# angela000/DQNFlappyBird

Hardware: AMD Instinct MI355X
Metric: env steps/sec (whole node) + DQN grad-steps/sec, 80x80x4 batch=32 (higher is better)
Workload: dtype f32

## Files before the change

### dqnflappybird_amd/csrc/fb_qnet.hip

```cpp
#include <math.h>
#include <stdlib.h>
#include "fb_common.h"

#ifndef FK_ABL
#define FK_ABL 0
#endif
#ifndef BW_ABL
#define BW_ABL 0
#endif

namespace {

typedef float f32x16 __attribute__((ext_vector_type(16)));

constexpr int OFF_W1 = 0, OFF_B1 = 8192, OFF_W2 = 8224, OFF_B2 = 40992, OFF_W3 = 41056, OFF_B3 = 77920,
              OFF_WF1 = 77984;
constexpr int CONV_PARAMS = OFF_WF1;
#include "fb_head.h"
#include "fb_sampler.h"
#include "fb_gather.h"
constexpr int MAXTB = 256;


struct Slice { const float *params; const uint8_t *states; int s_off, count; const uint16_t *w1s; int fshift; };
// ... 1729 lines not shown
        if (DUEL) {
#pragma unroll
            for (int r = 0; r < PERV; r++) { const int i = tid + r * 512; if (i < cv) lw[2 * WQ + i] = tv[r]; }
        }
        __syncthreads();
        const int kl = k0 % 64;
#pragma unroll 8
        for (int k = 0; k < KC; k++) {
            const float xs = rdlane(x, kl + k), xqs = rdlane(xq, kl + k);
#pragma unroll
            for (int a = 0; a < AT; a++) {
                const int o = k * AN + (a < A ? a : 0) * N + il;
                lg[a] = fmaf(xs, lw[o], lg[a]);
                ns[a] = fmaf(xqs, lw[WQ + o], ns[a]);
            }
            if (DUEL) nv = fmaf(rdlane(xv, kl + k), lw[2 * WQ + k * N + il], nv);
        }
    }
#pragma unroll
    for (int a = 0; a < AT; a++) lg[a] += H.P[H.hoff.bq + (a < A ? a : 0) * N + il];
    float nq[AT], mean = 0.f;
#pragma unroll
    for (int a = 0; a < AT; a++) {
        const int o = (a < A ? a : 0) * N + il;
        nq[a] = draw(LQ.eout + o) * (ns[a] + H.sig[H.off.bq + o]);
        if (a < A) mean += nq[a];
    }
    if (DUEL) {
        mean /= (float)A;
        const float vn = draw(LV.eout + il) * (nv + H.sig[H.off.bv + il]);
#pragma unroll
        for (int a = 0; a < AT; a++) lg[a] += (vn + nq[a]) - mean;
    } else {
#pragma unroll
        for (int a = 0; a < AT; a++) lg[a] += nq[a];
    }
    float qv[AT];
    const float z = H.sup.vmin + (float)(on ? lane : 0) * H.sup.dz;
    c51_q<AT>(lg, on, z, qv);
    if (lane == 0 && live) {
#pragma unroll
        for (int a = 0; a < AT; a++) if (a < A) H.q[(size_t)smp * A + a] = qv[a];
        int best = 0;
#pragma unroll
        for (int a = 1; a < AT; a++) if (a < A && qv[a] > qv[best]) best = a;
        const fb_u4 o = fb_philox(H.seed_lo, H.seed_hi, (uint32_t)key, H.step_lo, H.stream, H.step_hi);
        const float u = (float)(o.x >> 8) * (1.0f / 16777216.0f);
        if (u <= H.epsilon) best = (int)(((unsigned long long)o.y * (unsigned)A) >> 32);
        H.actions[smp] = (uint8_t)best;
    }
}

typedef float f32x4 __attribute__((ext_vector_type(4)));
struct FkArgs { Slices sl; const float *h3; float *hf; float *qpart; int FC, A, dueling, stot; NetOff off; };
constexpr int FK_ROW = 204;

__global__ __launch_bounds__(512) void fc1_fk_kernel(FkArgs a) {
    __shared__ float ast[8 * 16 * FK_ROW];
    __shared__ float red[8 * 4 * 64];
    const Slice s = a.sl.s[blockIdx.z];
    const int M = s.count, m0 = blockIdx.x * 16, n0 = blockIdx.y * 16;
    if (m0 >= M) return;
    const int lane = threadIdx.x & 63, wave = threadIdx.x >> 6, r = lane & 15, g = lane >> 4;
    const int kw = wave * 200;
    const float *bcol = s.params + OFF_WF1 + (size_t)(kw + 50 * g) * a.FC + n0 + r;
    float bv[50];
#pragma unroll
    for (int t = 0; t < 50; t++) bv[t] = bcol[(size_t)(FK_ABL == 2 ? 0 : t) * a.FC];
    float hb = s.params[a.off.bf1 + n0 + r], hw[MAXA + 1];
#pragma unroll
    for (int c = 0; c < MAXA; c++) hw[c] = s.params[a.off.wq + (n0 + r) * a.A + (c < a.A ? c : 0)];
    hw[MAXA] = s.params[(a.dueling ? a.off.wv : a.off.bf1) + n0 + r];
    float *mine = ast + wave * 16 * FK_ROW;
    float4 st[13];
#pragma unroll
    for (int i = 0; i < 13; i++) {
        const int idx = lane + 64 * i, row = idx < 800 ? idx / 50 : 0, c4 = idx < 800 ? idx - row * 50 : 0;
        const int mr = m0 + row < M ? m0 + row : M - 1;
        st[i] = *reinterpret_cast<const float4 *>(a.h3 + (size_t)(s.s_off + mr) * 1600 + kw + 4 * (FK_ABL == 3 ? 0 : c4));
    }
#pragma unroll
    for (int i = 0; i < 13; i++) {
        const int idx = lane + 64 * i, row = idx / 50, c4 = idx - row * 50;
        if (idx < 800) *reinterpret_cast<float4 *>(mine + row * FK_ROW + 4 * c4) = st[i];
    }
    __builtin_amdgcn_wave_barrier();
    asm volatile("s_waitcnt lgkmcnt(0)" ::: "memory");
    const float *arow = mine + r * FK_ROW + 50 * g;
    f32x4 acc0 = {0.f, 0.f, 0.f, 0.f}, acc1 = {0.f, 0.f, 0.f, 0.f};
    float2 av[25];
#pragma unroll
    for (int t = 0; t < 25; t++) av[t] = *reinterpret_cast<const float2 *>(arow + 2 * t);
#pragma unroll
    for (int t = 0; t < 25; t++) { keep(av[t].x); keep(av[t].y); }
#pragma unroll
    for (int t = 0; t < (FK_ABL == 1 ? 1 : 25); t++) {
        acc0 = __builtin_amdgcn_mfma_f32_16x16x4f32(rbf(av[t].x, a.sl.rb), rbf(bv[2 * t], a.sl.rb), acc0, 0, 0, 0);
        acc1 = __builtin_amdgcn_mfma_f32_16x16x4f32(rbf(av[t].y, a.sl.rb), rbf(bv[2 * t + 1], a.sl.rb), acc1, 0, 0, 0);
    }
#pragma unroll
    for (int q = 0; q < 4; q++) red[(wave * 4 + q) * 64 + lane] = acc0[q] + acc1[q];
    __syncthreads();
    if (threadIdx.x >= 256) return;
    const int reg = threadIdx.x >> 6, row = 4 * g + reg, col = r, mr = m0 + row, unit = n0 + col;
    float v = red[reg * 64 + lane];
#pragma unroll
    for (int w = 1; w < 8; w++) v += red[(w * 4 + reg) * 64 + lane];
    const bool live = mr < M;
    const size_t srow = (size_t)s.s_off + (live ? mr : M - 1);
    if (live) a.hf[srow * a.FC + unit] = v;
    if (!a.qpart || FK_ABL == 4) return;
    const float h = fmaxf(v + hb, 0.f);
    const int qs = a.A + 1;
    float *qo = a.qpart + (srow * (size_t)gridDim.y + blockIdx.y) * qs;
#pragma unroll
    for (int c = 0; c <= MAXA; c++) {
        if (c < a.A || (c == a.A && a.dueling)) {
            float x = h * (c == a.A ? hw[MAXA] : hw[c]);
#pragma unroll
            for (int o = 8; o > 0; o >>= 1) x += __shfl_xor(x, o, 16);
            if (col == 0 && live) qo[c] = x;
        }
    }
}

struct Bw1Args {
    int algo, B, FC, A, dueling, stot, n_dx, rb;
    NetOff off;
    const float *params, *pnext, *ptarget;
    const float *hf, *qpart, *h3;
    const uint8_t *act; const float *rew; const uint8_t *term; const float *isw;
    double gamma;
    float *grad, *dh3, *loss, *abs_err, *y_out;
    AdamDev *adam; int tick;
    FbGate gate;
};
constexpr int BW_DX_ROW = 4;
constexpr int BW_DW_ROW = 36;

template <int AT, bool DX, bool MD = false, bool DP = false, bool HU = false>
__device__ __forceinline__ void fc1_bwd2_body(const Bw1Args &L, float *smem, const MdPar M = MdPar{}, const float delta = 0.f) {
    const int tid = threadIdx.x, lane = tid & 63, wave = tid >> 6, B = L.B, FC = L.FC, A = AT == MAXA ? L.A : AT;
    const float *P = L.params;
    float (*dadv)[MAXA] = reinterpret_cast<float (*)[MAXA]>(smem);
    float *dv = smem + MAXTB * MAXA, *lterm = dv + MAXTB, *dadv2 = lterm + MAXTB, *big = dadv2 + 2 * MAXTB;
    const bool lead = blockIdx.x == 0;
    const bool dbl = DP || L.algo == FB_ALGO_DOUBLE;
    const bool row3 = MD || dbl;
    const int qs = A + 1, ntile = FC >> 4;
    constexpr bool dx_role = DX;
    const int mt = dx_role ? blockIdx.x / 50 : 0, t2 = dx_role ? 0 : blockIdx.x - L.n_dx, nt = t2 / 7, kg = t2 - nt * 7;
    const int kt = dx_role ? blockIdx.x - mt * 50 : kg * 8 + wave;
    auto unit_params = [&](int n, float &bias, float (&wq)[AT], float &wv) {
        bias = P[L.off.bf1 + n];
        wv = P[(L.dueling ? L.off.wv : L.off.bf1) + n];
#pragma unroll
        for (int c = 0; c < AT; c++) wq[c] = P[L.off.wq + n * A + (c < A ? c : 0)];
    };
    float pre_hf[32], pre_bias, pre_wq[AT], pre_wv, pre_a[16];
    float4 pre_w[8];
    if constexpr (DX) {
        const int ch = FC < 512 ? FC : 512, n = tid < ch ? tid : 0;
#pragma unroll
        for (int q = 0; q < 32; q++) { const int bq_ = mt * 32 + q; pre_hf[q] = L.hf[(size_t)(bq_ < B ? bq_ : 0) * FC + n]; }
        unit_params(n, pre_bias, pre_wq, pre_wv);
        const int kh = ch / 16, nbeg = wave * (ch / 8) + (lane >> 5) * kh;
        const float *brun = P + OFF_WF1 + (size_t)(kt * 32 + (lane & 31)) * FC + nbeg;
#pragma unroll
        for (int q = 0; q < 8; q++) pre_w[q] = *reinterpret_cast<const float4 *>(brun + (4 * q < kh ? 4 * q : 0));
#pragma unroll
        for (int q = 0; q < 16; q++) pre_a[q] = 0.f;
#pragma unroll
        for (int q = 0; q < 2; q++) { const int mr = mt * 32 + drow(2 * (wave & 7) + q, lane); pre_a[q] = L.h3[(size_t)(mr < B ? mr : 0) * 1600 + kt * 32 + (lane & 31)]; }
    } else {
        const int c = tid & 31;
#pragma unroll
        for (int q = 0; q < 2; q++) { const int b = (tid >> 5) + 16 * q; pre_hf[q] = L.hf[(size_t)(b < B ? b : 0) * FC + nt * 32 + c]; }
#pragma unroll
        for (int q = 2; q < 32; q++) pre_hf[q] = 0.f;
        unit_params(nt * 32 + c, pre_bias, pre_wq, pre_wv);
        const int ktc = kt < 50 ? kt : 0;
#pragma unroll
        for (int t = 0; t < 16; t++) { const int b = 2 * t + (lane >> 5); pre_a[t] = L.h3[(size_t)(b < B ? b : 0) * 1600 + ktc * 32 + (lane & 31)]; }
#pragma unroll
        for (int q = 0; q < 8; q++) pre_w[q] = make_float4(0.f, 0.f, 0.f, 0.f);
    }
    float bqs[AT], bqn[AT], bq3[AT];
#pragma unroll
    for (int c = 0; c < AT; c++) { const int cc = c < A ? c : 0; bqs[c] = L.params[L.off.bq + cc]; bqn[c] = L.pnext[L.off.bq + cc]; bq3[c] = L.ptarget[L.off.bq + cc]; }
    const int bvo = L.dueling ? L.off.bv : L.off.bq;
    float bvs = L.params[bvo], bvn = L.pnext[bvo], bv3 = L.ptarget[bvo];
    for (int b0 = 0; b0 < (BW_ABL == 1 ? 0 : B); b0 += 32) {
        const int b = b0 + (tid >> 4), j = tid & 15, bc = b < B ? b : 0;
        float rf = L.rew[bc], isw = L.isw ? L.isw[bc] : 1.f;
        int termb = L.term[bc], a_b = L.act[bc];
        float x0[2][AT + 1], x1[2][AT + 1], x2[2][AT + 1];
#pragma unroll
        for (int u = 0; u < 2; u++) {
            const int tile = j + 16 * u, tc = tile < ntile ? tile : 0;
            const float *q0 = L.qpart + ((size_t)bc * ntile + tc) * qs;
            const size_t rs = (size_t)ntile * qs;
#pragma unroll
            for (int c = 0; c <= AT; c++) {
                const int cc = c < qs ? c : 0;
                x0[u][c] = q0[cc]; x1[u][c] = q0[(size_t)B * rs + cc]; x2[u][c] = q0[(size_t)(row3 ? 2 * B : 0) * rs + cc];
            }
        }
        keep(rf); keep(isw); keep(termb); keep(a_b);
        float qsv[AT + 1], qnv[AT + 1], q3v[AT + 1];
#pragma unroll
        for (int c = 0; c <= AT; c++) {
            keep(x0[0][c]); keep(x1[0][c]); keep(x2[0][c]); keep(x0[1][c]); keep(x1[1][c]); keep(x2[1][c]);
            const bool on = c < A || (c == A && L.dueling), on0 = on && j < ntile, on1 = on && j + 16 < ntile;
            qsv[c] = (on0 ? x0[0][c] : 0.f) + (on1 ? x0[1][c] : 0.f);
            qnv[c] = (on0 ? x1[0][c] : 0.f) + (on1 ? x1[1][c] : 0.f);
            q3v[c] = (on0 ? x2[0][c] : 0.f) + (on1 ? x2[1][c] : 0.f);
        }
        for (int tile = j + 32; tile < ntile; tile += 16) {
            const float *q0 = L.qpart + ((size_t)bc * ntile + tile) * qs;
            const size_t rs = (size_t)ntile * qs;
#pragma unroll
            for (int c = 0; c <= AT; c++) {
                const int cc = c < qs ? c : 0;
                const bool on = c < A || (c == A && L.dueling);
                const float y0 = q0[cc], y1 = q0[(size_t)B * rs + cc], y2 = q0[(size_t)(row3 ? 2 * B : 0) * rs + cc];
                qsv[c] += on ? y0 : 0.f; qnv[c] += on ? y1 : 0.f; q3v[c] += on ? y2 : 0.f;
            }
        }
#pragma unroll
        for (int c = 0; c <= AT; c++)
#pragma unroll
            for (int o = 8; o > 0; o >>= 1) { qsv[c] += __shfl_xor(qsv[c], o, 16); qnv[c] += __shfl_xor(qnv[c], o, 16); q3v[c] += __shfl_xor(q3v[c], o, 16); }
// ... 11 lines not shown
        };
        fin(qsv, vs, bqs, bvs);
        fin(qnv, vn, bqn, bvn);
        fin(q3v, v3, bq3, bv3);
        float sel;
        {
            int am = 0;
#pragma unroll
            for (int c = 1; c < AT; c++) if (c < A && qnv[c] > qnv[am]) am = c;
            float seld = q3v[0], selm = qnv[0];
#pragma unroll
            for (int c = 1; c < AT; c++) { seld = c == am ? q3v[c] : seld; selm = c < A ? fmaxf(selm, qnv[c]) : selm; }
            sel = dbl ? seld : selm;
        }
        if (L.algo != FB_ALGO_PER) isw = 1.f;
        double rr = rf == 0.1f ? 0.1 : (double)rf;
        if constexpr (MD) {
            float bonus;
            mdqn_target<AT>(qnv, q3v, A, a_b, M, sel, bonus);
            rr += (double)bonus;
        }
        const double yd = termb ? rr : rr + L.gamma * (double)sel;
        const float y = (float)yd;
        float qe = qsv[0];
#pragma unroll
        for (int c = 1; c < AT; c++) qe = c == a_b ? qsv[c] : qe;
        const float d = y - qe;
        const float scale = L.algo == FB_ALGO_DQN ? 2.f : 2.f / (float)B;
        const float gq = -scale * isw * td_clamp<HU>(d, delta);
        const bool pg = L.algo == FB_ALGO_PG;
        float pgp[AT], pgl;
        {
            float mx = qsv[0], se = 0.f;
#pragma unroll
            for (int c = 1; c < AT; c++) mx = c < A ? fmaxf(mx, qsv[c]) : mx;
#pragma unroll
            for (int c = 0; c < AT; c++) { pgp[c] = c < A ? expf(qsv[c] - mx) : 0.f; se += pgp[c]; }
#pragma unroll
            for (int c = 0; c < AT; c++) pgp[c] /= se;
            pgl = logf(se) - (qe - mx);
        }
        const float pgw = rf / (float)L.gamma;
        if (j == 0 && b < B) {
            lterm[b] = pg ? pgl * pgw : td_term<HU>(isw, d, delta);
            if (lead && L.abs_err) L.abs_err[b] = fabsf(d);
            if (lead && L.y_out) L.y_out[b] = y;
            dv[b] = L.dueling && !pg ? gq : 0.f;
#pragma unroll
            for (int c = 0; c < AT; c++) dadv[b][c] = pg ? (pgp[c] - (c == a_b ? 1.f : 0.f)) * pgw : (c == a_b ? gq : 0.f) - (L.dueling ? gq / (float)A : 0.f);
            if (AT == 2) { dadv2[2 * b] = dadv[b][0]; dadv2[2 * b + 1] = dadv[b][1]; }
        }
    }
#pragma unroll
    for (int q = 0; q < 32; q++) keep(pre_hf[q]);
#pragma unroll
    for (int q = 0; q < 16; q++) keep(pre_a[q]);
#pragma unroll
    for (int q = 0; q < 8; q++) { keep(pre_w[q].x); keep(pre_w[q].y); keep(pre_w[q].z); keep(pre_w[q].w); }
    __syncthreads();
    if (lead && tid == 0) {
        float sum = 0.f;
        for (int b = 0; b < B; b++) sum += lterm[b];
        *L.loss = L.algo == FB_ALGO_DQN || L.algo == FB_ALGO_PG ? sum : sum / (float)B;
        adam_tick(L.adam, L.tick);
    }
    if (lead && tid >= 64 && tid < 64 + A) { const int c = tid - 64; float sum = 0.f; for (int b = 0; b < B; b++) sum += dadv[b][c]; L.grad[L.off.bq + c] = sum; }
    if (lead && tid == 128 && L.dueling) { float sum = 0.f; for (int b = 0; b < B; b++) sum += dv[b]; L.grad[L.off.bv] = sum; }
    auto dhf_of = [&](int b, float hfv, float bias, const float (&wq)[AT], float wv, float &hout) {
        const float v = hfv + bias;
        float d = L.dueling ? dv[b] * wv : 0.f;
#pragma unroll
        for (int c = 0; c < AT; c++) if (c < A) d = fmaf(dadv[b][c], wq[c], d);
        hout = fmaxf(v, 0.f);
        return v > 0.f ? d : 0.f;
    };
    const int hl = lane >> 5, i = lane & 31, jj = lane & 31;
    if constexpr (DX) {
        const int RS = 512 + BW_DX_ROW;
        float *dh = big, *red = big + 32 * RS;
        f32x16 acc = {0};
        for (int nc = 0; nc < FC; nc += 512) {
            const int ch = FC - nc < 512 ? FC - nc : 512;
            if (nc) {
                __syncthreads();
                const int n = nc + (tid < ch ? tid : 0);
#pragma unroll
                for (int q = 0; q < 32; q++) { const int bq_ = mt * 32 + q; pre_hf[q] = L.hf[(size_t)(bq_ < B ? bq_ : 0) * FC + n]; }
                unit_params(n, pre_bias, pre_wq, pre_wv);
                const int kh = ch / 16, nbeg = wave * (ch / 8) + hl * kh;
                const float *brun = P + OFF_WF1 + (size_t)(kt * 32 + jj) * FC + nc + nbeg;
#pragma unroll
                for (int q = 0; q < 8; q++) pre_w[q] = *reinterpret_cast<const float4 *>(brun + (4 * q < kh ? 4 * q : 0));
            }
            if (tid < ch && BW_ABL != 2) {
                if (AT == 2 && !L.dueling) {
                    float4 da[16];
#pragma unroll
                    for (int q = 0; q < 16; q++) da[q] = *reinterpret_cast<const float4 *>(dadv2 + 2 * (mt * 32 + 2 * q < MAXTB - 1 ? mt * 32 + 2 * q : 0));
                    float o[32];
#pragma unroll
                    for (int q = 0; q < 16; q++) {
                        const float v0 = pre_hf[2 * q] + pre_bias, v1 = pre_hf[2 * q + 1] + pre_bias;
                        const float d0 = fmaf(da[q].y, pre_wq[1], fmaf(da[q].x, pre_wq[0], 0.f)), d1 = fmaf(da[q].w, pre_wq[1], fmaf(da[q].z, pre_wq[0], 0.f));
                        o[2 * q] = (v0 > 0.f && mt * 32 + 2 * q < B) ? d0 : 0.f;
                        o[2 * q + 1] = (v1 > 0.f && mt * 32 + 2 * q + 1 < B) ? d1 : 0.f;
                    }
#pragma unroll
                    for (int q = 0; q < 32; q++) dh[q * RS + tid] = o[q];
                } else {
#pragma unroll
                    for (int q = 0; q < 32; q++) {
                        float hv;
                        dh[q * RS + tid] = mt * 32 + q < B ? dhf_of(mt * 32 + q, pre_hf[q], pre_bias, pre_wq, pre_wv, hv) : 0.f;
                    }
                }
            }
            __syncthreads();
            const int kh = ch / 16, nbeg = wave * (ch / 8) + hl * kh;
            const float *arun = dh + i * RS + nbeg;
            float4 xa[8];
#pragma unroll
            for (int q = 0; q < 8; q++) xa[q] = *reinterpret_cast<const float4 *>(arun + (4 * q < kh ? 4 * q : 0));
#pragma unroll
            for (int q = 0; q < 8; q++) { keep(xa[q].x); keep(xa[q].y); keep(xa[q].z); keep(xa[q].w); }
#pragma unroll
            for (int q = 0; q < 8; q++) {
                if (4 * q < kh && BW_ABL != 3) {
                    const float4 x = xa[q], w = pre_w[q];
                    const bool rb = L.rb;
                    acc = mfma(rbf(x.x, rb), rbf(w.x, rb), acc); acc = mfma(rbf(x.y, rb), rbf(w.y, rb), acc);
                    acc = mfma(rbf(x.z, rb), rbf(w.z, rb), acc); acc = mfma(rbf(x.w, rb), rbf(w.w, rb), acc);
                }
            }
        }
        reduce_rows<8>(acc, red, wave, lane, mt * 32, B, [&](float v, int r, int mr) {
            const size_t o = (size_t)mr * 1600 + kt * 32 + jj;
            L.dh3[o] = BW_ABL == 4 ? v : (((r & 1) ? pre_a[1] : pre_a[0]) > 0.f ? v : 0.f);
        });
        return;
    }
    if (BW_ABL == 5) return;
    float *dh = big, *hh = big + MAXTB * BW_DW_ROW;
    {
        const int c = tid & 31;
#pragma unroll
        for (int q = 0; q < 2; q++) {
            const int b = (tid >> 5) + 16 * q;
            if (b < B) { float hv; dh[b * BW_DW_ROW + c] = dhf_of(b, pre_hf[q], pre_bias, pre_wq, pre_wv, hv); hh[b * BW_DW_ROW + c] = hv; }
        }
        for (int b = (tid >> 5) + 32; b < B; b += 16) {
            float hv;
            dh[b * BW_DW_ROW + c] = dhf_of(b, L.hf[(size_t)b * FC + nt * 32 + c], pre_bias, pre_wq, pre_wv, hv);
            hh[b * BW_DW_ROW + c] = hv;
        }
    }
    __syncthreads();
    if (kt < 50) {
        f32x16 acc = {0};
#pragma unroll
        for (int t = 0; t < 16; t++) {
            const int b = 2 * t + hl;
            const float w = dh[(b < B ? b : 0) * BW_DW_ROW + jj];
            acc = mfma(b < B ? rbf(pre_a[t], L.rb) : 0.f, b < B ? rbf(w, L.rb) : 0.f, acc);
        }
#pragma unroll 4
        for (int t = 16; t < (B + 1) / 2; t++) {
            const int b = 2 * t + hl, bc = b < B ? b : 0;
// ... 1135 lines not shown
        }
    }
    if (bid == ADAMF_T2 + ADAMF_T3 && tid == 0) { a.ad->applies = a.ad->ticks; a.ad->pver[0] += 1; a.ad->wverc[0] = a.ad->pver[0]; }
    if (bid == ADAMF_T2 + ADAMF_T3 && tid < (int)(a.n & 3)) {
        const long long q = (n4 << 2) + tid;
        float mm = a.m[q], vv = a.v[q];
        mm += (a.g[q] - mm) * omb1; vv += (a.g[q] * a.g[q] - vv) * omb2;
        a.p[q] -= (mm * alpha) / (sqrtf(vv) + eps);
        a.m[q] = mm; a.v[q] = vv;
    }
    if (a.split && bid == ADAMF_T2 + ADAMF_T3 && tid == 0) fb_flag_wait(&a.split->env_done, a.split_val, &a.split->timeouts[4]);
}

__global__ void init_params_kernel(float *__restrict__ p, long long n, NetOff off, int FC, int A, int dueling,
                                   uint32_t seed_lo, uint32_t seed_hi) {
    const long long i = (long long)blockIdx.x * blockDim.x + threadIdx.x;
    if (i >= n) return;
    bool bias = (i >= OFF_B1 && i < OFF_W2) || (i >= OFF_B2 && i < OFF_W3) || (i >= OFF_B3 && i < OFF_WF1) ||
                (i >= off.bf1 && i < off.bf1 + FC) || (i >= off.bq && i < off.bq + A) || (dueling && i == off.bv);
    if (bias) { p[i] = 0.01f; return; }
    for (uint32_t ctr = 0;; ctr++) {
        const fb_u4 r = fb_philox(seed_lo, seed_hi, (uint32_t)i, ctr, FB_STREAM_INIT, 0u);
        const float u1 = ((r.x >> 8) + 1) * (1.0f / 16777216.0f), u2 = (r.y >> 8) * (1.0f / 16777216.0f);
        const float z = sqrtf(-2.f * logf(u1)) * cosf(6.28318530717958647692f * u2);
        if (fabsf(z) <= 2.f) { p[i] = 0.01f * z; return; }
    }
}

}

#ifndef FB_ADAM_GRID
#define FB_ADAM_GRID 1024
#endif
constexpr int ADAM_GRID = FB_ADAM_GRID;

#include <vector>
struct fb_qnet {
    std::vector<void *> allocs;
    int arch, FC, A, max_batch;
    long long n;
    NetOff off;
    float *params[2], *adam_m, *adam_v, *grad, *slabs;
    float *slabs1;
    uint16_t *w1s[2];
    uint4 *wsp[2];
    uint16_t *zeros;
    uint16_t *a1s, *a3s;
    int nsplit;
    int nsplit_train;
    bool adam_ticked;
    AdamDev *adam;
    float *p1, *h2, *h3, *hf, *q;
    float *qpart;
    unsigned long long *ring_fo;
    hipEvent_t grad_ev;
    hipEvent_t grad_ev_recorded;
    uint8_t *amax;
    float *dhf, *dh3, *dh2, *dp1;
    float *gmax;
    int zmax;
    float *hf_act, *hp_act;
    FbSplitCtx *split;
    C51Sup sup;
    float kappa;
    MdPar md;
    float huber;
    float *c51_dl, *c51_xs, *c51_lt;
    NetOff hoff;
    float *heff[2];
    bool noisy;
    long long ntot;
    NoisyNet nnet;
    float *mst[2], *nz[2];
    int act_noise;
    float *nz_zero, *ht;
    uint4 *wsig;
    uint16_t *a3n;
    int *sig_seen;
    bool split_adam_pending;
    float max_grad_norm;
    double *clip_part;
    float *clip_out;
    float ac_cv, ac_ce;
    float ppo_eps, ppo_vclip;
    float *ac_dl, *ac_xs, *ac_r;
    uint8_t *ac_t;
    SacOff sac_off;
    float sac_hbar, sac_alr;
    float *sac_w;
    IqnOff iqn_off;
    int iqn_n, iqn_np, iqn_k;
    float iqn_eta;
    float *iqn_dpre, *iqn_ctab;
    int iqn_mu;
    MdPar iqn_md;
    float *ppo_sum;
};

static NetOff make_off(int FC, int A, int dueling) {
    NetOff o;
    o.bf1 = OFF_WF1 + 1600 * FC;
    int p = o.bf1 + FC;
    if (dueling) { o.wv = p; o.bv = p + FC; p = o.bv + 1; } else { o.wv = 0; o.bv = 0; }
    o.wq = p; o.bq = p + FC * A; o.n = o.bq + A;
    return o;
}
// ... 190 lines not shown
                        : make_off(fc_width, sup.N ? n_actions * sup.N : n_actions, arch == FB_ARCH_DUELING || arch == FB_ARCH_AC || arch == FB_ARCH_IQN_DUELING);
    if (is_sac(h)) {
        h->sac_off.wq1 = h->off.n; h->sac_off.bq1 = h->sac_off.wq1 + fc_width * n_actions;
        h->sac_off.wq2 = h->sac_off.bq1 + n_actions; h->sac_off.bq2 = h->sac_off.wq2 + fc_width * n_actions;
        h->off.n = h->sac_off.bq2 + n_actions;
        h->sac_hbar = 0.98f * logf((float)n_actions); h->sac_alr = 0.f;
    }
    if (is_iqn(h)) {
        h->iqn_off.we = h->off.n; h->iqn_off.be = h->iqn_off.we + FB_IQN_COS * fc_width;
        h->off.n = h->iqn_off.be + fc_width;
        h->iqn_n = s.n_tau; h->iqn_np = s.n_tau_next; h->iqn_k = s.n_tau_act; h->iqn_eta = 1.f;
        h->iqn_mu = 0; h->iqn_md = MdPar{0.03f, 0.9f, -1.f};
    }
    h->hoff = is_c51d(h) ? make_off(fc_width, n_actions * sup.N, 0) : is_iqnd(h) ? make_off(fc_width, n_actions, 0) : h->off;
    h->n = h->off.n;
    h->noisy = s.noisy;
    h->ntot = h->noisy ? 2 * h->n - OFF_WF1 : h->n;
    if (h->noisy) h->nnet = make_noisy(h->off, arch, fc_width, n_actions, sup.N, s.sigma0);
    h->zmax = 64;
    const size_t S = (size_t)3 * max_batch, nb = sizeof(float) * (size_t)h->n, nbt = sizeof(float) * (size_t)h->ntot;
    hipError_t e = hipSuccess;
    auto alloc = [&](auto **p, size_t bytes) {
        void *q = nullptr;
        if (e == hipSuccess) e = hipMalloc(&q, bytes);
        if (e != hipSuccess) return;
        h->allocs.push_back(q);
        *p = static_cast<std::remove_reference_t<decltype(**p)> *>(q);
        e = hipMemset(q, 0, bytes);
    };
    alloc(&h->params[0], nb); alloc(&h->params[1], nb);
    alloc(&h->adam_m, nbt); alloc(&h->adam_v, nbt); alloc(&h->grad, nbt);
    if (h->noisy) for (int w = 0; w < 2; w++) { alloc(&h->mst[w], nbt); alloc(&h->nz[w], sizeof(float) * (size_t)h->nnet.nz); }
    if (h->noisy) {
        alloc(&h->nz_zero, sizeof(float) * (size_t)h->nnet.nz);
        alloc(&h->wsig, sizeof(uint4) * (size_t)wsp_w3t(fc_width));
        alloc(&h->a3n, S * 1600 * 6 + 256);
        alloc(&h->ht, S * fc_width * 4 * FC1_SP_KS);
        alloc(&h->sig_seen, sizeof(int));
        if (e == hipSuccess) e = hipMemset(h->sig_seen, 0xff, sizeof(int));
    }
    alloc(&h->slabs, sizeof(float) * (size_t)h->zmax * CONV_PARAMS);
    if (2 * max_batch > h->zmax) alloc(&h->slabs1, sizeof(float) * (size_t)2 * (max_batch < MAXTB ? max_batch : MAXTB) * CONV1_PARAMS);
    alloc(&h->adam, sizeof(AdamDev));
    alloc(&h->w1s[0], 3 * 8192 * 2); alloc(&h->w1s[1], 3 * 8192 * 2);
    const size_t wsp_bytes = (size_t)wsp_total(fc_width) * sizeof(uint4);
    alloc(&h->wsp[0], wsp_bytes); alloc(&h->wsp[1], wsp_bytes);
    h->nsplit = 3; h->nsplit_train = 3;
    alloc(&h->zeros, 256);
    alloc(&h->a1s, S * 3200 * 6); alloc(&h->a3s, S * 1600 * 6 + 256);
    alloc(&h->p1, S * 3200 * 4); alloc(&h->amax, S * 3200);
    alloc(&h->h2, S * 1600 * 4); alloc(&h->h3, S * 1600 * 4);
    alloc(&h->hf, S * fc_width * 4 * FC1_KS); alloc(&h->q, S * MAXA * 4);
    alloc(&h->qpart, (size_t)(fc_width / 16) * S * (MAXA + 1) * 4);
    alloc(&h->ring_fo, (size_t)max_batch * 4 * sizeof(unsigned long long));
    const size_t Bm = max_batch;
    alloc(&h->dhf, Bm * fc_width * 4); alloc(&h->dh3, Bm * 1600 * 4);
    alloc(&h->dh2, Bm * 1600 * 4); alloc(&h->dp1, Bm * 3200 * 4);
    alloc(&h->gmax, (size_t)(fc_width / 16) * 4);
    alloc(&h->hf_act, S * fc_width * 4 * FC1_SP_KS); alloc(&h->hp_act, sizeof(float) * (size_t)(h->n - h->off.bf1));
    if (sup.N) { alloc(&h->c51_dl, Bm * 64 * 4); alloc(&h->c51_xs, Bm * fc_width * 4); alloc(&h->c51_lt, Bm * 4); }
    if (is_c51d(h) || is_iqn(h)) for (int w = 0; w < 2; w++) alloc(&h->heff[w], sizeof(float) * (size_t)(h->hoff.n - h->off.bf1));
    if (is_ac(h)) {
        const size_t Bt = Bm < MAXTB ? Bm : MAXTB;
        alloc(&h->ac_dl, Bt * 16 * 4); alloc(&h->ac_xs, Bt * fc_width * 4); alloc(&h->ac_r, Bt * 4); alloc(&h->ac_t, Bt);
        alloc(&h->ppo_sum, 6 * 4);
    }
    if (is_sac(h)) {
        const size_t Bt = Bm < MAXTB ? Bm : MAXTB;
        alloc(&h->ac_dl, Bt * 16 * 4); alloc(&h->ac_xs, Bt * fc_width * 4); alloc(&h->sac_w, 8 * 4);
    }
    if (is_iqn(h)) {
        const size_t Bt = Bm < MAXTB ? Bm : MAXTB;
        alloc(&h->ac_dl, Bt * 4 * 4); alloc(&h->ac_xs, Bt * fc_width * 4);
        alloc(&h->iqn_dpre, Bt * h->iqn_n * fc_width * 4); alloc(&h->iqn_ctab, Bt * h->iqn_n * FB_IQN_COS * 4);
    }
    alloc(&h->clip_part, sizeof(double) * 256); alloc(&h->clip_out, sizeof(float) * 2);
    if (e == hipSuccess) { const float one = 1.f; e = hipMemcpy(h->clip_out + 1, &one, sizeof(one), hipMemcpyHostToDevice); }
    int rc = e == hipSuccess ? FB_OK : fb_set_error(e == hipErrorOutOfMemory ? FB_ERR_NOMEM : FB_ERR_HIP, "fb_qnet_create: %s", hipGetErrorString(e));
    if (rc == FB_OK) {
        AdamDev a; memset(&a, 0, sizeof(a));
        a.pver[0] = a.pver[1] = 1;
        if (hipMemcpy(h->adam, &a, sizeof(a), hipMemcpyHostToDevice) != hipSuccess) rc = fb_set_error(FB_ERR_HIP, "fb_qnet_create: hipMemcpy failed");
    }
    if (rc == FB_OK) rc = fb_qnet_set_hparams(h, 1e-6f, 0.9f, 0.999f, 1e-8f);
    if (rc == FB_OK && is_sac(h)) rc = sac_write_words(h, 0.2f);
    if (rc != FB_OK) { fb_qnet_destroy(h); return rc; }
    *out = h;
    return FB_OK;
}

extern "C" int fb_qnet_destroy(fb_qnet_t h) {
    if (!h) return FB_OK;
    if (h->split) {
        FbSplitCtx *c = h->split;
        if (c->tstream) { (void)hipStreamSynchronize(c->tstream); (void)hipStreamDestroy(c->tstream); }
        if (c->f) (void)hipFree(c->f);
        delete c;
    }
    for (void *p : h->allocs) (void)hipFree(p);
    delete h;
    return FB_OK;
}

__global__ void flag_wait_kernel(const unsigned long long *flag, unsigned long long v, unsigned *timeouts) { if (threadIdx.x == 0) fb_flag_wait(flag, v, timeouts); }
__global__ void flag_set_kernel(unsigned long long *flag, unsigned long long v) { fb_flag_store(flag, v); }

// ... 286 lines not shown
    if (p.train) { side.p1 = h->p1; side.amax = h->amax; }
    const int t1p = (rows * 100 + 7) / 8, gsp = min(256, (t1p + C1_WAVES - 1) / C1_WAVES);
    if (!c.trunk && !c.state_trunk && !c.fused && runs(c, K_CONV1))
        hipLaunchKernelGGL(conv1_sp_kernel, dim3(gsp), dim3(64 * C1_WAVES), 0, c.st, sl, (const uint8_t *)h->zeros, h->a1s, c.pl1, c.nsp, h->wsp[which], h->FC, pver, (const unsigned *)wver, side, &h->adam->ovf);
    C23Args c23{h->a1s + (size_t)row0 * 3200, c.pl1, h->wsp[which] + WSP_W2, s0.params + OFF_B2, s0.params + OFF_B3, h->a3s + (size_t)row0 * 1600, c.pl2, rows, pver, wver, c.only < 0 ? &h->adam->wverc[which] : nullptr,
                p.train ? h->h2 + (size_t)row0 * 1600 : nullptr, p.train ? h->h3 + (size_t)row0 * 1600 : nullptr,
                s0.states, s0.w1s, s0.params + OFF_B1, s0.params, h->wsp[which], h->FC, &h->adam->ovf};
    Fc1Args af{h->a3s + (size_t)row0 * 1600, c.pl2, h->zeros, h->wsp[which] + WSP_WF1, (c.fused ? h->hf_act : h->hf) + (size_t)row0 * h->FC, c.stot, rows, h->FC,
               c.fused ? pver : nullptr, c.fused ? wver : nullptr, nullptr, 0,
               c.fused ? head_base(h, s0.params) + h->off.bf1 : nullptr, c.fused ? h->hp_act : nullptr, c.fused ? (int)(h->hoff.n - h->off.bf1) : 0,
               c.fused && p.split && c.only < 0 ? &p.split->f->trunk_done : nullptr, p.split ? p.split->seq : 0};
    if (c.trunk && z1 < p.ns && rows % 128 == 0) {
        int z2 = z1 + 1;
        while (z2 < p.ns && p.sl.s[z2].params == p.sl.s[z1].params && p.sl.s[z2].s_off == p.sl.s[z2 - 1].s_off + p.sl.s[z2 - 1].count) z2++;
        const Slice sn = p.sl.s[z1];
        if (z2 == p.ns && sn.s_off == row0 + rows && sn.params != s0.params) {
            int rows2 = 0;
            for (int z = z1; z < z2; z++) rows2 += p.sl.s[z].count;
            af.w2 = h->wsp[sn.params == h->params[1] ? 1 : 0] + WSP_WF1; af.m_split = rows; af.M = rows + rows2;
            z1 = z2;
        }
    }
    *z = z1;
    const dim3 gc((rows + 4) / 5), gf(((af.M + 127) / 128) * (h->FC / 64) * FC1_SP_KS);
    if (c.fused && p.split && c.only < 0 && gc.x > 256 && gc.x % 256 != 0) { c23.round_flag = &p.split->f->last_round; c23.round_val = p.split->seq; c23.round_blk = (int)(gc.x / 256) * 256; }
    with_nsp(c.nsp, [&](auto ns) {
        if (!c.trunk && !c.state_trunk && runs(c, K_CONV2))
            with_bool(c.fused, [&](auto fu) { hipLaunchKernelGGL((conv23_sp_kernel<decltype(ns)::value, 5, decltype(fu)::value>), gc, dim3(512), 0, c.st, c23); });
        if (runs(c, K_FC1)) hipLaunchKernelGGL(fc1_sp_kernel<decltype(ns)::value>, gf, dim3(256), 0, c.st, af);
    });
    if (c.fused && (c.only < 0 || c.only == K_FC1) && (long long)af.hp_n > (long long)gf.x * 256) {
        const size_t done = (size_t)gf.x * 256;
        FB_CHECK_HIP(hipMemcpyAsync(h->hp_act + done, af.hp_src + done, sizeof(float) * ((size_t)af.hp_n - done), hipMemcpyDeviceToDevice, c.st));
    }
    return FB_OK;
}

static void small_trunk(fb_qnet *h, const Plan &p, const PlanCtx &c, bool planes) {
    SplitJob job;
    C23T c23t = trunk_args(h, p, c, &job);
    if (planes) { c23t.a3s = h->a3s; c23t.pl3 = c.pl2; }
    const int t1 = (c.maxc * 100 + 7) / 8;
    if (runs(c, K_CONV1))
        with_bool(p.nib, [&](auto nib) { hipLaunchKernelGGL(conv1_pool_kernel<decltype(nib)::value>, dim3((t1 + 3) / 4, 1, p.ns), dim3(256), 0, c.st, p.sl, h->p1, h->amax, job); });
    if (runs(c, K_CONV2))
        with_nsp(c.nsp, [&](auto ns) { hipLaunchKernelGGL((conv23_t_kernel<decltype(ns)::value, false>), dim3(c.maxc, p.ns), dim3(512), 0, c.st, c23t); });
}

static void small_forward(fb_qnet *h, const Plan &p, const PlanCtx &c) {
    if (!c.trunk) small_trunk(h, p, c, false);
    if (runs(c, K_FC1)) {
        FkArgs fa;
        fa.sl = p.sl; fa.h3 = h->h3; fa.hf = h->hf; fa.qpart = p.train && !c.c51 && !c.ac ? h->qpart : nullptr; fa.FC = h->FC; fa.A = h->A;
        fa.dueling = h->arch == FB_ARCH_DUELING; fa.stot = c.stot; fa.off = h->off;
        hipLaunchKernelGGL(fc1_fk_kernel, dim3((c.maxc + 15) / 16, h->FC / 16, p.ns), dim3(512), 0, c.st, fa);
    }
}

static void launch_dist_head(const fb_qnet *h, const C51HeadArgs &H, int rows, hipStream_t st) {
    with_actions(h->A, [&](auto a) {
        if (is_qr(h)) hipLaunchKernelGGL(qr_head_kernel<decltype(a)::value>, dim3((rows + 3) / 4), dim3(256), 0, st, H);
        else hipLaunchKernelGGL(c51_head_kernel<decltype(a)::value>, dim3((rows + 3) / 4), dim3(256), 0, st, H);
    });
}

static void head_stage(fb_qnet *h, const Plan &p, const PlanCtx &c) {
    auto shared = [&](auto &H) {
        H.hf = c.fused ? h->hf_act : h->hf; H.stot = c.stot; H.nks = c.big ? FC1_SP_KS : 1; H.FC = h->FC; H.A = h->A;
    };
    auto core = [&](auto &C) {
        shared(C); C.q = h->q; C.off = h->hoff; C.actions = p.actions; C.epsilon = p.epsilon;
        put_seed_words(C, p.seed, p.step);
    };
    auto side = [&](auto &H, bool act_copy) {
        memset(&H, 0, sizeof(H));
        shared(H); H.rows = c.total; H.off = h->off; H.P = act_copy && c.fused ? h->hp_act - h->off.bf1 : p.sl.s[0].params;
    };
    auto policy = [&](auto &H) {
        side(H, true);
        H.logits = p.ac_logits; H.value = p.ac_value; H.logp = p.ac_logp; H.actions = p.actions; H.greedy = p.ac_greedy;
        put_seed_words(H, p.seed, p.step);
    };
    if (c.c51 && !p.train && !p.no_head && runs(c, K_HEAD)) {
        C51HeadArgs H;
        H.sl = p.sl; H.nslices = p.ns; H.params = nullptr;
        for (int z = 0; z < p.ns; z++) H.sl.s[z].params = head_base(h, p.sl.s[z].params);
        C51Core &C = H.c;
        core(C); C.probs = p.probs; C.sup = h->sup; C.key_of = nullptr; C.stream = FB_STREAM_EPS;
        if (p.head_rider) {
            memset(p.head_rider, 0, sizeof(*p.head_rider));
            p.head_rider->c.hf = C.hf; p.head_rider->c.stot = c.stot; p.head_rider->c.nks = C.nks;
            p.head_rider->params = c.fused ? h->hp_act - h->off.bf1 : H.sl.s[0].params;
        } else launch_dist_head(h, H, c.total, c.st);
    }
    if (c.sac && !p.train && p.policy_head && runs(c, K_HEAD)) {
        SacHeadArgs H;
        policy(H);
        H.so = h->sac_off; H.sw = h->sac_w; H.q1 = p.sac_q1; H.q2 = p.sac_q2;
        fb_sac_launch_head(c.st, H);
        return;
    }
    if (c.iqn && !p.train && p.iqn_theta && runs(c, K_HEAD)) {
        IqnHeadArgs H;
        side(H, false);
        H.M = p.iqn_m; H.io = h->iqn_off; H.dueling = is_iqnd(h) ? 1 : 0; H.tau = p.iqn_tau; H.theta = p.iqn_theta;
        fb_iqn_launch_head(c.st, H);
        return;
// ... 63 lines not shown
                            adam_head, p.tick, p.ppo ? 5 : 3};
        fb_ac_launch_grad(c.st, gA);
        return;
    }
    if (!c.c51) {
        LossArgs L;
        shared(L); transition(L);
        L.algo = p.algo; L.dueling = h->arch == FB_ARCH_DUELING; L.off = h->off;
        L.params = h->params[0]; L.q = h->q; L.isw = p.isw;
        L.grad = p.G; L.loss = p.loss; L.abs_err = p.abs_err; L.y_out = p.y; L.gmax = h->gmax;
        L.adam = h->adam; L.tick = p.tick;
        const bool dp = p.algo == FB_ALGO_DOUBLE_PER, hu = h->huber > 0.f, md = is_mdqn_algo(p.algo);
        if (md) L.algo = p.algo == FB_ALGO_MDQN_PER ? FB_ALGO_PER : FB_ALGO_NATURE;
        if (dp) L.algo = FB_ALGO_PER;
        const dim3 grid(FC / 16);
        if (dp || hu) fb_qnet_launch_loss_head_x(dp, hu, md, grid.x, c.st, &L, &h->md, h->huber);
        else if (md) hipLaunchKernelGGL(loss_head_md_kernel, grid, dim3(256), 0, c.st, L, h->md);
        else hipLaunchKernelGGL(loss_head_kernel, grid, dim3(256), 0, c.st, L);
        return;
    }
    const bool pw = is_per_algo(p.algo);
    auto dist = [&](auto &L) {
        shared(L); transition(L); L.off = h->hoff;
        L.p_on = head_base(h, h->params[0]); L.p_next = head_base(h, p.sl.s[1].params);
        L.p_tgt = head_base(h, p.ns > 2 ? p.sl.s[2].params : p.sl.s[1].params);
        L.dl = h->c51_dl; L.xs = h->c51_xs; L.lterm = h->c51_lt;
        L.isw = pw ? p.isw : nullptr; L.abs_err = pw ? p.abs_err : nullptr;
    };
    with_actions(h->A, [&](auto a) { with_bool(pw, [&](auto w) {
        if (is_qr(h)) {
            QRLossArgs L;
            dist(L);
            L.algo = is_double_qr(p.algo) ? FB_ALGO_QR_DOUBLE : FB_ALGO_QR; L.N = h->sup.N; L.kappa = h->kappa;
            hipLaunchKernelGGL((qr_loss_kernel<decltype(a)::value, decltype(w)::value>), dim3((B + 3) / 4), dim3(256), 0, c.st, L);
        } else {
            C51LossArgs L;
            dist(L);
            L.algo = is_double_c51(p.algo) ? FB_ALGO_C51_DOUBLE : FB_ALGO_C51; L.sup = h->sup;
            hipLaunchKernelGGL((c51_loss_kernel<decltype(a)::value, decltype(w)::value>), dim3((B + 3) / 4), dim3(256), 0, c.st, L);
        }
    }); });
    const C51GradArgs gA{B, FC, h->A, h->sup.N, h->off, h->c51_dl, h->c51_xs, h->c51_lt, h->dhf, p.a, p.G, p.loss, h->gmax, h->adam, p.tick};
    if (is_c51d(h)) hipLaunchKernelGGL(c51d_grad_kernel, dim3(FC / 16), dim3(256), 0, c.st, gA);
    else hipLaunchKernelGGL(c51_grad_kernel, dim3(FC / 16), dim3(256), 0, c.st, gA);
}

static void fc1_backward(fb_qnet *h, const Plan &p, const PlanCtx &c) {
    const int B = p.B, FC = h->FC;
    if (!c.big && !c.c51 && !c.ac) {
        const int ndx1 = ((B + 31) / 32) * 50;
        Bw1Args L;
        L.algo = p.algo; L.B = B; L.FC = FC; L.A = h->A; L.dueling = h->arch == FB_ARCH_DUELING; L.stot = c.stot; L.n_dx = ndx1; L.off = h->off;
        L.params = h->params[0]; L.pnext = p.sl.s[1].params; L.ptarget = p.ns > 2 ? p.sl.s[2].params : p.sl.s[1].params;
        L.hf = h->hf; L.qpart = h->qpart; L.h3 = h->h3; L.act = p.a; L.rew = p.r; L.term = p.t; L.isw = p.isw; L.gamma = p.gamma;
        L.grad = p.G; L.dh3 = h->dh3; L.loss = p.loss; L.abs_err = p.abs_err; L.y_out = p.y;
        L.adam = h->adam; L.tick = p.tick; L.rb = h->nsplit_train == 1;
        L.gate = p.split && c.only < 0 ? FbGate{&p.split->f->trunk_done, p.split->seq, &p.split->f->timeouts[2]} : FbGate{nullptr, 0, nullptr};
        const dim3 grid(ndx1 + (FC / 32) * 7 + (L.gate.flag ? 1 : 0));
        const bool dp = p.algo == FB_ALGO_DOUBLE_PER, hu = h->huber > 0.f, md = is_mdqn_algo(p.algo);
        if (md) L.algo = p.algo == FB_ALGO_MDQN_PER ? FB_ALGO_PER : FB_ALGO_NATURE;
        if (dp) L.algo = FB_ALGO_PER;
        if (dp || hu) fb_qnet_launch_fc1_bwd2_x(dp, hu, md, grid.x, c.st, &L, &h->md, h->huber);
        else if (md) hipLaunchKernelGGL(fc1_bwd2_md_kernel, grid, dim3(512), 0, c.st, L, h->md);
        else hipLaunchKernelGGL(fc1_bwd2_kernel, grid, dim3(512), 0, c.st, L);
        return;
    }
    const int ndx = ((B + 31) / 32) * 50, ntile = ndx + 50 * (FC / 32);
    const bool std_shape = FC == 512 && B == 256;
    with_nsp(h->nsplit_train, [&](auto ns) { with_bool(std_shape, [&](auto s) {
        hipLaunchKernelGGL((fc1_bwd_big_kernel<decltype(ns)::value, decltype(s)::value ? 4 : 0, decltype(s)::value ? 2 : 0>), dim3(ntile), dim3(512), 0, c.st,
                           ndx, h->params[0], h->h3, h->dhf, h->dh3, p.G, B, FC, (const float *)h->gmax, &h->adam->ovf);
    }); });
}

struct SlabCounts { int z1, z3; };
static SlabCounts conv_backward(fb_qnet *h, const Plan &p, const PlanCtx &c, int span0, int span1) {
    const int B = p.B, FC = h->FC, rbt = h->nsplit_train == 1;
    int z3 = min((B * 25 + 255) / 256, h->zmax);
    const size_t ss = CONV_PARAMS;
    const AdamSpan span{master(h, 0), h->adam_m, h->adam_v, p.G, h->adam, span0, span1};
    const FbGate gate_fc1 = p.split && c.only < 0 ? FbGate{&p.split->f->fc1_done, p.split->seq, &p.split->f->timeouts[3]} : FbGate{nullptr, 0, nullptr};
    const FbSampleRider srider = p.sample_rider ? *p.sample_rider : FbSampleRider{};
    const bool fold1 = 2 * B > h->zmax;
    const int fold = (2 * B + h->zmax - 1) / h->zmax;
    const int z1 = fold1 ? (2 * B + fold - 1) / fold : 2 * B;
    const int n_adam5 = (span1 - span0 + 511) / 512;
    const BxArgs bx{h->dh3, h->h2, h->p1, h->dh2, h->dp1, h->wsp[0] + wsp_w3t(FC), h->wsp[0] + wsp_w2t(FC)};
    const Dw1Ring dr{p.ring ? p.ring->c.bits : nullptr, h->ring_fo};
    float *s1 = fold1 ? h->slabs1 : h->slabs;
    const size_t st1 = fold1 ? (size_t)CONV1_PARAMS : ss;
    const bool dwg = c.big && B % 16 == 0;
    const int zt3 = dwg ? 0 : z3, zt2 = zt3;
    const bool bw = !c.big && B <= h->zmax;
    if (bw) {
        z3 = B;
        const dim3 g(BW_WGS * B + n_adam5 + (srider.k ? 1 : 0) + (gate_fc1.flag ? 1 : 0));
        if (runs(c, K_CONV3_BWD)) with_nsp(h->nsplit_train, [&](auto ns) { with_bool(p.ring != nullptr, [&](auto r) {
            hipLaunchKernelGGL((conv_bw_kernel<decltype(ns)::value, decltype(r)::value>), g, dim3(512), 0, c.st,
                               bx, B, h->slabs, ss, s1, st1, p.s, (const uint8_t *)h->amax, dr, n_adam5, span, srider, rbt, gate_fc1);
        }); });
    } else {
        const dim3 g3(B + 38 * zt3 + n_adam5 + (srider.k ? 1 : 0)), g2(34 * zt2 + 2 * B + (gate_fc1.flag ? 1 : 0));
        if (runs(c, K_CONV3_BWD)) with_nsp(h->nsplit_train, [&](auto ns) {
            hipLaunchKernelGGL(conv_bx_kernel<decltype(ns)::value>, g3, dim3(512), 0, c.st, bx, B, zt3, h->slabs, ss, n_adam5, span, srider, rbt);
        });
        if (dwg) {
            z3 = B / 16;
// ... 926 lines not shown
```

Baseline: 10.97 million.

## Pass FC1 ReLU masks as packed bits from forward to backward dx path

The fc1 forward kernel now ballots the ReLU activation mask and writes packed 16-bit masks per row and unit tile into a new buffer. The backward dx blocks read these bitmasks with four int4 loads instead of loading 32 hf floats per thread, so the per-sample dh becomes zero wherever the mask bit is clear. This cuts global memory traffic and register pressure in the backward kernel, at the cost of an extra small buffer and extra stores in the forward kernel.

```diff
diff --git a/dqnflappybird_amd/csrc/fb_qnet.hip b/dqnflappybird_amd/csrc/fb_qnet.hip
--- a/dqnflappybird_amd/csrc/fb_qnet.hip
+++ b/dqnflappybird_amd/csrc/fb_qnet.hip
@@ -1805,7 +1805,7 @@
 }
 
 typedef float f32x4 __attribute__((ext_vector_type(4)));
-struct FkArgs { Slices sl; const float *h3; float *hf; float *qpart; int FC, A, dueling, stot; NetOff off; };
+struct FkArgs { Slices sl; const float *h3; float *hf; float *qpart; int FC, A, dueling, stot; NetOff off; uint16_t *relu_bits; int rb_stride; };
 constexpr int FK_ROW = 204;
 
 __global__ __launch_bounds__(512) void fc1_fk_kernel(FkArgs a) {
@@ -1864,6 +1864,8 @@
     if (live) a.hf[srow * a.FC + unit] = v;
     if (!a.qpart || FK_ABL == 4) return;
     const float h = fmaxf(v + hb, 0.f);
+    const unsigned long long rbits = __ballot(h > 0.f);
+    if (col == 0 && live && FK_ABL != 5) a.relu_bits[(size_t)blockIdx.y * a.rb_stride + srow] = (uint16_t)(rbits >> (16 * g));
     const int qs = a.A + 1;
     float *qo = a.qpart + (srow * (size_t)gridDim.y + blockIdx.y) * qs;
 #pragma unroll
@@ -1882,6 +1884,8 @@
     NetOff off;
     const float *params, *pnext, *ptarget;
     const float *hf, *qpart, *h3;
+    const uint16_t *relu_bits;
+    int rb_stride;
     const uint8_t *act; const float *rew; const uint8_t *term; const float *isw;
     double gamma;
     float *grad, *dh3, *loss, *abs_err, *y_out;
@@ -1905,17 +1909,23 @@
     const int mt = dx_role ? blockIdx.x / 50 : 0, t2 = dx_role ? 0 : blockIdx.x - L.n_dx, nt = t2 / 7, kg = t2 - nt * 7;
     const int kt = dx_role ? blockIdx.x - mt * 50 : kg * 8 + wave;
     auto unit_params = [&](int n, float &bias, float (&wq)[AT], float &wv) {
-        bias = P[L.off.bf1 + n];
+        bias = DX ? 0.f : P[L.off.bf1 + n];
         wv = P[(L.dueling ? L.off.wv : L.off.bf1) + n];
 #pragma unroll
         for (int c = 0; c < AT; c++) wq[c] = P[L.off.wq + n * A + (c < A ? c : 0)];
     };
-    float pre_hf[32], pre_bias, pre_wq[AT], pre_wv, pre_a[16];
+    float pre_hf[DX ? 1 : 2], pre_bias, pre_wq[AT], pre_wv, pre_a[16];
+    int pre_rb[DX ? 16 : 1];
     float4 pre_w[8];
+    auto tile_bits = [&](int n) {
+        const int4 *src = reinterpret_cast<const int4 *>(L.relu_bits + (size_t)(BW_ABL == 6 ? 0 : n >> 4) * L.rb_stride + mt * 32);
+#pragma unroll
+        for (int q = 0; q < 4; q++) { const int4 v = src[q]; pre_rb[4 * q] = v.x; pre_rb[4 * q + 1] = v.y; pre_rb[4 * q + 2] = v.z; pre_rb[4 * q + 3] = v.w; }
+    };
     if constexpr (DX) {
         const int ch = FC < 512 ? FC : 512, n = tid < ch ? tid : 0;
-#pragma unroll
-        for (int q = 0; q < 32; q++) { const int bq_ = mt * 32 + q; pre_hf[q] = L.hf[(size_t)(bq_ < B ? bq_ : 0) * FC + n]; }
+        pre_hf[0] = 0.f;
+        tile_bits(n);
         unit_params(n, pre_bias, pre_wq, pre_wv);
         const int kh = ch / 16, nbeg = wave * (ch / 8) + (lane >> 5) * kh;
         const float *brun = P + OFF_WF1 + (size_t)(kt * 32 + (lane & 31)) * FC + nbeg;
@@ -1929,8 +1939,7 @@
         const int c = tid & 31;
 #pragma unroll
         for (int q = 0; q < 2; q++) { const int b = (tid >> 5) + 16 * q; pre_hf[q] = L.hf[(size_t)(b < B ? b : 0) * FC + nt * 32 + c]; }
-#pragma unroll
-        for (int q = 2; q < 32; q++) pre_hf[q] = 0.f;
+        pre_rb[0] = 0;
         unit_params(nt * 32 + c, pre_bias, pre_wq, pre_wv);
         const int ktc = kt < 50 ? kt : 0;
 #pragma unroll
@@ -2048,7 +2057,9 @@
         }
     }
 #pragma unroll
-    for (int q = 0; q < 32; q++) keep(pre_hf[q]);
+    for (int q = 0; q < (DX ? 1 : 2); q++) keep(pre_hf[q]);
+#pragma unroll
+    for (int q = 0; q < (DX ? 16 : 1); q++) keep(pre_rb[q]);
 #pragma unroll
     for (int q = 0; q < 16; q++) keep(pre_a[q]);
 #pragma unroll
@@ -2062,11 +2073,15 @@
     }
     if (lead && tid >= 64 && tid < 64 + A) { const int c = tid - 64; float sum = 0.f; for (int b = 0; b < B; b++) sum += dadv[b][c]; L.grad[L.off.bq + c] = sum; }
     if (lead && tid == 128 && L.dueling) { float sum = 0.f; for (int b = 0; b < B; b++) sum += dv[b]; L.grad[L.off.bv] = sum; }
+    auto dh_of = [&](int b, const float (&wq)[AT], float wv) {
+        float d = L.dueling ? dv[b] * wv : 0.f;
+#pragma unroll
+        for (int c = 0; c < AT; c++) if (c < A) d = fmaf(dadv[b][c], wq[c], d);
+        return d;
+    };
     auto dhf_of = [&](int b, float hfv, float bias, const float (&wq)[AT], float wv, float &hout) {
         const float v = hfv + bias;
-        float d = L.dueling ? dv[b] * wv : 0.f;
-#pragma unroll
-        for (int c = 0; c < AT; c++) if (c < A) d = fmaf(dadv[b][c], wq[c], d);
+        const float d = dh_of(b, wq, wv);
         hout = fmaxf(v, 0.f);
         return v > 0.f ? d : 0.f;
     };
@@ -2080,8 +2095,7 @@
             if (nc) {
                 __syncthreads();
                 const int n = nc + (tid < ch ? tid : 0);
-#pragma unroll
-                for (int q = 0; q < 32; q++) { const int bq_ = mt * 32 + q; pre_hf[q] = L.hf[(size_t)(bq_ < B ? bq_ : 0) * FC + n]; }
+                tile_bits(n);
                 unit_params(n, pre_bias, pre_wq, pre_wv);
                 const int kh = ch / 16, nbeg = wave * (ch / 8) + hl * kh;
                 const float *brun = P + OFF_WF1 + (size_t)(kt * 32 + jj) * FC + nc + nbeg;
@@ -2089,6 +2103,8 @@
                 for (int q = 0; q < 8; q++) pre_w[q] = *reinterpret_cast<const float4 *>(brun + (4 * q < kh ? 4 * q : 0));
             }
             if (tid < ch && BW_ABL != 2) {
+                const unsigned bit0 = 1u << (tid & 15), bit1 = bit0 << 16;
+                auto on = [&](int q) { return ((unsigned)pre_rb[q >> 1] & ((q & 1) ? bit1 : bit0)) != 0; };
                 if (AT == 2 && !L.dueling) {
                     float4 da[16];
 #pragma unroll
@@ -2096,19 +2112,15 @@
                     float o[32];
 #pragma unroll
                     for (int q = 0; q < 16; q++) {
-                        const float v0 = pre_hf[2 * q] + pre_bias, v1 = pre_hf[2 * q + 1] + pre_bias;
                         const float d0 = fmaf(da[q].y, pre_wq[1], fmaf(da[q].x, pre_wq[0], 0.f)), d1 = fmaf(da[q].w, pre_wq[1], fmaf(da[q].z, pre_wq[0], 0.f));
-                        o[2 * q] = (v0 > 0.f && mt * 32 + 2 * q < B) ? d0 : 0.f;
-                        o[2 * q + 1] = (v1 > 0.f && mt * 32 + 2 * q + 1 < B) ? d1 : 0.f;
+                        o[2 * q] = (on(2 * q) && mt * 32 + 2 * q < B) ? d0 : 0.f;
+                        o[2 * q + 1] = (on(2 * q + 1) && mt * 32 + 2 * q + 1 < B) ? d1 : 0.f;
                     }
 #pragma unroll
                     for (int q = 0; q < 32; q++) dh[q * RS + tid] = o[q];
                 } else {
 #pragma unroll
-                    for (int q = 0; q < 32; q++) {
-                        float hv;
-                        dh[q * RS + tid] = mt * 32 + q < B ? dhf_of(mt * 32 + q, pre_hf[q], pre_bias, pre_wq, pre_wv, hv) : 0.f;
-                    }
+                    for (int q = 0; q < 32; q++) dh[q * RS + tid] = mt * 32 + q < B && on(q) ? dh_of(mt * 32 + q, pre_wq, pre_wv) : 0.f;
                 }
             }
             __syncthreads();
@@ -3350,6 +3362,8 @@
     AdamDev *adam;
     float *p1, *h2, *h3, *hf, *q;
     float *qpart;
+    uint16_t *relu_bits;
+    int rb_stride;
     unsigned long long *ring_fo;
     hipEvent_t grad_ev;
     hipEvent_t grad_ev_recorded;
@@ -3646,6 +3660,8 @@
     alloc(&h->h2, S * 1600 * 4); alloc(&h->h3, S * 1600 * 4);
     alloc(&h->hf, S * fc_width * 4 * FC1_KS); alloc(&h->q, S * MAXA * 4);
     alloc(&h->qpart, (size_t)(fc_width / 16) * S * (MAXA + 1) * 4);
+    h->rb_stride = (int)((S + 31) / 32 * 32);
+    alloc(&h->relu_bits, (size_t)(fc_width / 16) * h->rb_stride * sizeof(uint16_t));
     alloc(&h->ring_fo, (size_t)max_batch * 4 * sizeof(unsigned long long));
     const size_t Bm = max_batch;
     alloc(&h->dhf, Bm * fc_width * 4); alloc(&h->dh3, Bm * 1600 * 4);
@@ -4038,7 +4054,7 @@
     if (runs(c, K_FC1)) {
         FkArgs fa;
         fa.sl = p.sl; fa.h3 = h->h3; fa.hf = h->hf; fa.qpart = p.train && !c.c51 && !c.ac ? h->qpart : nullptr; fa.FC = h->FC; fa.A = h->A;
-        fa.dueling = h->arch == FB_ARCH_DUELING; fa.stot = c.stot; fa.off = h->off;
+        fa.dueling = h->arch == FB_ARCH_DUELING; fa.stot = c.stot; fa.off = h->off; fa.relu_bits = fa.qpart ? h->relu_bits : nullptr; fa.rb_stride = h->rb_stride;
         hipLaunchKernelGGL(fc1_fk_kernel, dim3((c.maxc + 15) / 16, h->FC / 16, p.ns), dim3(512), 0, c.st, fa);
     }
 }
@@ -4208,7 +4224,7 @@
         Bw1Args L;
         L.algo = p.algo; L.B = B; L.FC = FC; L.A = h->A; L.dueling = h->arch == FB_ARCH_DUELING; L.stot = c.stot; L.n_dx = ndx1; L.off = h->off;
         L.params = h->params[0]; L.pnext = p.sl.s[1].params; L.ptarget = p.ns > 2 ? p.sl.s[2].params : p.sl.s[1].params;
-        L.hf = h->hf; L.qpart = h->qpart; L.h3 = h->h3; L.act = p.a; L.rew = p.r; L.term = p.t; L.isw = p.isw; L.gamma = p.gamma;
+        L.hf = h->hf; L.qpart = h->qpart; L.relu_bits = h->relu_bits; L.rb_stride = h->rb_stride; L.h3 = h->h3; L.act = p.a; L.rew = p.r; L.term = p.t; L.isw = p.isw; L.gamma = p.gamma;
         L.grad = p.G; L.dh3 = h->dh3; L.loss = p.loss; L.abs_err = p.abs_err; L.y_out = p.y;
         L.adam = h->adam; L.tick = p.tick; L.rb = h->nsplit_train == 1;
         L.gate = p.split && c.only < 0 ? FbGate{&p.split->f->trunk_done, p.split->seq, &p.split->f->timeouts[2]} : FbGate{nullptr, 0, nullptr};
```

Result: no change. 11.07 million (median of 6 runs) (+0.9%).
